# Xjh-UCAS/TAM-TR

Measured on AMD Instinct MI355X. Metric: images/sec fwd+bwd @640x640 bs=16/GPU, higher is better.
Workload: dtype bf16

## Files before the change

### tam-tr_amd/csrc/dwconv.hip

```cpp
#include "common.h"

namespace {

constexpr int TS = 16;
constexpr int DW_THREADS = TS * TS;
#ifndef DW_CB_BWD
#define DW_CB_BWD 16
#endif
constexpr int CB_FWD = 32, CB_BWD = DW_CB_BWD;

__device__ __forceinline__ float silu_f(float v) { return v / (1.f + __expf(-v)); }

template <typename T>
struct Vec16;
template <>
struct Vec16<float> {
  static constexpr int N = 4;
  static __device__ __forceinline__ void ld(const float* p, float (&o)[4]) {
    const float4 v = *reinterpret_cast<const float4*>(p);
    o[0] = v.x; o[1] = v.y; o[2] = v.z; o[3] = v.w;
  }
  static __device__ __forceinline__ void st(float* p, const float (&v)[4]) { *reinterpret_cast<float4*>(p) = make_float4(v[0], v[1], v[2], v[3]); }
};
template <>
struct Vec16<bf16_t> {
  static constexpr int N = 8;
  static __device__ __forceinline__ void ld(const bf16_t* p, float (&o)[8]) {
    const uint4 v = *reinterpret_cast<const uint4*>(p);
    const uint32_t w[4] = {v.x, v.y, v.z, v.w};
#pragma unroll
    for (int i = 0; i < 4; ++i) { o[2 * i] = __uint_as_float(w[i] << 16); o[2 * i + 1] = __uint_as_float(w[i] & 0xffff0000u); }
  }
  static __device__ __forceinline__ void st(bf16_t* p, const float (&v)[8]) {
    uint4 o;
    o.x = (uint32_t)f2bf(v[0]) | ((uint32_t)f2bf(v[1]) << 16); o.y = (uint32_t)f2bf(v[2]) | ((uint32_t)f2bf(v[3]) << 16);
    o.z = (uint32_t)f2bf(v[4]) | ((uint32_t)f2bf(v[5]) << 16); o.w = (uint32_t)f2bf(v[6]) | ((uint32_t)f2bf(v[7]) << 16);
    *reinterpret_cast<uint4*>(p) = o;
  }
};

__device__ __forceinline__ void plane_st(float* p, float v) { *p = v; }
__device__ __forceinline__ void plane_st(bf16_t* p, float v) { *p = f2bf(v); }
__device__ __forceinline__ float plane_ld(const float* p) { return *p; }
__device__ __forceinline__ float plane_ld(const bf16_t* p) { return bf2f(*p); }
__device__ __forceinline__ float4 plane_ld4(const float* p) { return *reinterpret_cast<const float4*>(p); }
__device__ __forceinline__ float4 plane_ld4(const bf16_t* p) {
  const uint2 v = *reinterpret_cast<const uint2*>(p);
  return make_float4(__uint_as_float(v.x << 16), __uint_as_float(v.x & 0xffff0000u), __uint_as_float(v.y << 16), __uint_as_float(v.y & 0xffff0000u));
}

template <typename T, int CB, int HALO, int PITCH>
__device__ __forceinline__ void stage_tile(const T* __restrict__ x, size_t xs, int b, int d0, int h0, int w0, int H, int W,
                                           float (*s)[TS + 2 * HALO][PITCH]) {
  constexpr int SIDE = TS + 2 * HALO, VN = Vec16<T>::N, GROUPS = CB / VN, TOTAL = SIDE * SIDE * GROUPS;
  constexpr int N_IT = (TOTAL + DW_THREADS - 1) / DW_THREADS;
  float v[N_IT][VN];
#pragma unroll
  for (int k = 0; k < N_IT; ++k) {
    const int it = min((int)threadIdx.x + k * DW_THREADS, TOTAL - 1);
    const int pix = it / GROUPS, gq = it - pix * GROUPS;
    const int py = pix / SIDE, px = pix - py * SIDE;
    const int h = min(max(h0 + py - HALO, 0), H - 1), w = min(max(w0 + px - HALO, 0), W - 1);
    Vec16<T>::ld(x + ((size_t)(b * H + h) * W + w) * xs + d0 + gq * VN, v[k]);
  }
#pragma unroll
  for (int k = 0; k < N_IT; ++k) {
    const int it = threadIdx.x + k * DW_THREADS;
    if (it < TOTAL) {
      const int pix = it / GROUPS, gq = it - pix * GROUPS;
      const int py = pix / SIDE, px = pix - py * SIDE;
      const int h = h0 + py - HALO, w = w0 + px - HALO;
      const float keep = (h >= 0 && h < H && w >= 0 && w < W) ? 1.f : 0.f;
#pragma unroll
      for (int j = 0; j < VN; ++j) s[gq * VN + j][py][px] = v[k][j] * keep;
    }
  }
}

template <typename T, typename PT>
__global__ __launch_bounds__(DW_THREADS) void dwconv_cross_fwd_kernel(const T* __restrict__ x, size_t xs, const float* __restrict__ wgt,
                                                                       const float* __restrict__ bias, PT* __restrict__ u2, int D,
                                                                       int H, int W, int tiles_w) {
  constexpr int CB = CB_FWD, SIDE = TS + 2, PITCH = SIDE + 1;
  __shared__ float s_in[CB][SIDE][PITCH];
  __shared__ float s_w[CB][10];
  const int th = blockIdx.x / tiles_w, tw = blockIdx.x - th * tiles_w;
  const int d0 = blockIdx.y * CB, b = blockIdx.z, h0 = th * TS, w0 = tw * TS;
  const size_t L = (size_t)H * W;
  for (int i = threadIdx.x; i < CB * 10; i += DW_THREADS) {
    const int c = i / 10, k = i - c * 10;
    s_w[c][k] = k < 9 ? wgt[(size_t)(d0 + c) * 9 + k] : (bias ? bias[d0 + c] : 0.f);
  }
  stage_tile<T, CB, 1, PITCH>(x, xs, b, d0, h0, w0, H, W, s_in);
  __syncthreads();
#pragma unroll
  for (int pass = 0; pass < 2; ++pass) {
    const int ty = pass == 0 ? threadIdx.x / TS : threadIdx.x % TS;
    const int tx = pass == 0 ? threadIdx.x % TS : threadIdx.x / TS;
    const int h = h0 + ty, w = w0 + tx;
    if (h >= H || w >= W) continue;
    PT* out = u2 + ((size_t)(b * 2 + pass) * D + d0) * L + (pass == 0 ? (size_t)h * W + w : (size_t)w * H + h);
    for (int c = 0; c < CB; ++c) {
      float acc = s_w[c][9];
#pragma unroll
      for (int ky = 0; ky < 3; ++ky)
#pragma unroll
        for (int kx = 0; kx < 3; ++kx) acc = fmaf(s_w[c][ky * 3 + kx], s_in[c][ty + ky][tx + kx], acc);
      plane_st(out + (size_t)c * L, silu_f(acc));
    }
  }
}

template <typename T, typename PT>
__global__ __launch_bounds__(DW_THREADS) void dwconv_cross_bwd_kernel(const PT* __restrict__ g2, const T* __restrict__ x, size_t xs,
                                                                       const float* __restrict__ wgt, const float* __restrict__ bias,
                                                                       T* __restrict__ gx, size_t gxs, float* __restrict__ ws, int D,
                                                                       int H, int W, int tiles_w, int tiles) {
  constexpr int CB = CB_BWD, XS = TS + 4, XP = XS + 1, GS = TS + 2, GP = GS + 1;
  __shared__ float s_x[CB][XS][XP];
  __shared__ float s_g[CB][GS][GP];
  __shared__ float s_w[CB][10];
  const int th = blockIdx.x / tiles_w, tw = blockIdx.x - th * tiles_w;
  const int d0 = blockIdx.y * CB, b = blockIdx.z, h0 = th * TS, w0 = tw * TS;
  const size_t L = (size_t)H * W;
  for (int i = threadIdx.x; i < CB * 10; i += DW_THREADS) {
    const int c = i / 10, k = i - c * 10;
    s_w[c][k] = k < 9 ? wgt[(size_t)(d0 + c) * 9 + k] : (bias ? bias[d0 + c] : 0.f);
  }
#ifndef DW_ABL_NOX
  stage_tile<T, CB, 2, XP>(x, xs, b, d0, h0, w0, H, W, s_x);
#endif
#ifndef DW_ABL_NOG
  if ((W & 3) == 0 && (H & 3) == 0) {
    constexpr int NV = 6, ITEMS_V = CB * GS * NV, N_ITV = (ITEMS_V + DW_THREADS - 1) / DW_THREADS;
#pragma unroll
    for (int plane = 0; plane < 2; ++plane) {
      const PT* gp = g2 + ((size_t)(b * 2 + plane) * D + d0) * L;
      float4 v[N_ITV];
#pragma unroll
      for (int k = 0; k < N_ITV; ++k) {
        const int it = min((int)threadIdx.x + k * DW_THREADS, ITEMS_V - 1);
        const int c = it / (GS * NV), r = it - c * (GS * NV), line = r / NV, q = r - line * NV;
        const int fixed = (plane == 0 ? h0 : w0) + line - 1, base = (plane == 0 ? w0 : h0) - 4 + 4 * q;
        const int nfix = plane == 0 ? H : W, nrun = plane == 0 ? W : H;
        const bool ok = fixed >= 0 && fixed < nfix && base >= 0 && base + 3 < nrun;
        const float4 t = plane_ld4(gp + (size_t)c * L + (size_t)min(max(fixed, 0), nfix - 1) * nrun + min(max(base, 0), nrun - 4));
        const float f = ok ? 1.f : 0.f;
        v[k] = make_float4(t.x * f, t.y * f, t.z * f, t.w * f);
      }
      if (plane == 1) __syncthreads();
#pragma unroll
      for (int k = 0; k < N_ITV; ++k) {
        const int it = threadIdx.x + k * DW_THREADS;
        if (it < ITEMS_V) {
          const int c = it / (GS * NV), r = it - c * (GS * NV), line = r / NV, q = r - line * NV;
          const float e[4] = {v[k].x, v[k].y, v[k].z, v[k].w};
#pragma unroll
          for (int j = 0; j < 4; ++j) {
            const int pos = 4 * q + j - 3;
            if (pos >= 0 && pos < GS) {
              if (plane == 0) s_g[c][line][pos] = e[j];
              else s_g[c][pos][line] += e[j];
            }
          }
        }
      }
    }
  } else {
  {
    constexpr int GB = 7, N_IT = ((CB * GS * GS + DW_THREADS - 1) / DW_THREADS + GB - 1) / GB * GB;
    const PT* gp = g2 + ((size_t)(b * 2 + 0) * D + d0) * L;
#pragma unroll 1
    for (int k0 = 0; k0 < N_IT; k0 += GB) {
      float v[GB];
#pragma unroll
      for (int k = 0; k < GB; ++k) {
        const int it = min((int)threadIdx.x + (k0 + k) * DW_THREADS, CB * GS * GS - 1);
        const int c = it / (GS * GS), r = it - c * (GS * GS), py = r / GS, px = r - py * GS;
        const int h = h0 + py - 1, w = w0 + px - 1;
        const bool ok = h >= 0 && h < H && w >= 0 && w < W;
        v[k] = plane_ld(gp + (size_t)c * L + (size_t)min(max(h, 0), H - 1) * W + min(max(w, 0), W - 1)) * (ok ? 1.f : 0.f);
      }
#pragma unroll
      for (int k = 0; k < GB; ++k) {
        const int it = threadIdx.x + (k0 + k) * DW_THREADS;
        if (it < CB * GS * GS) {
          const int c = it / (GS * GS), r = it - c * (GS * GS), py = r / GS, px = r - py * GS;
          s_g[c][py][px] = v[k];
        }
      }
    }
  }
  __syncthreads();
  {
    constexpr int GB = 7, N_IT = ((CB * GS * GS + DW_THREADS - 1) / DW_THREADS + GB - 1) / GB * GB;
    const PT* gp = g2 + ((size_t)(b * 2 + 1) * D + d0) * L;
#pragma unroll 1
    for (int k0 = 0; k0 < N_IT; k0 += GB) {
      float v[GB];
#pragma unroll
      for (int k = 0; k < GB; ++k) {
        const int it = min((int)threadIdx.x + (k0 + k) * DW_THREADS, CB * GS * GS - 1);
        const int c = it / (GS * GS), r = it - c * (GS * GS), px = r / GS, py = r - px * GS;
        const int h = h0 + py - 1, w = w0 + px - 1;
        const bool ok = h >= 0 && h < H && w >= 0 && w < W;
        v[k] = plane_ld(gp + (size_t)c * L + (size_t)min(max(w, 0), W - 1) * H + min(max(h, 0), H - 1)) * (ok ? 1.f : 0.f);
      }
#pragma unroll
      for (int k = 0; k < GB; ++k) {
        const int it = threadIdx.x + (k0 + k) * DW_THREADS;
        if (it < CB * GS * GS) {
          const int c = it / (GS * GS), r = it - c * (GS * GS), px = r / GS, py = r - px * GS;
          s_g[c][py][px] += v[k];
        }
      }
    }
  }
  }
#endif
  __syncthreads();
#ifndef DW_ABL_NOSILU
  {
    constexpr int TPC = DW_THREADS / CB;
    static_assert(DW_THREADS % CB == 0 && TPC <= WAVE && (TPC & (TPC - 1)) == 0, "a power-of-two lane group per channel");
    const int c = threadIdx.x / TPC, sub = threadIdx.x % TPC;
    float wk[9], dwk[10];
#pragma unroll
    for (int k9 = 0; k9 < 9; ++k9) { wk[k9] = s_w[c][k9]; dwk[k9] = 0.f; }
    dwk[9] = 0.f;
    const float bc = s_w[c][9];
    for (int r = sub; r < GS * GS; r += TPC) {
      const int px = r / GS, py = r - px * GS;
      const int h = h0 + py - 1, w = w0 + px - 1;
      float g = 0.f;
      if (h >= 0 && h < H && w >= 0 && w < W) {
        g = s_g[c][py][px];
        float xin[9], acc = bc;
#pragma unroll
        for (int ky = 0; ky < 3; ++ky)
#pragma unroll
          for (int kx = 0; kx < 3; ++kx) { xin[ky * 3 + kx] = s_x[c][py + ky][px + kx]; acc = fmaf(wk[ky * 3 + kx], xin[ky * 3 + kx], acc); }
        const float sg = 1.f / (1.f + __expf(-acc));
        g *= sg * (1.f + acc * (1.f - sg));
        if (py >= 1 && py <= TS && px >= 1 && px <= TS) {
#pragma unroll
          for (int k9 = 0; k9 < 9; ++k9) dwk[k9] = fmaf(g, xin[k9], dwk[k9]);
          dwk[9] += g;
        }
      }
      s_g[c][py][px] = g;
    }
#pragma unroll
    for (int k9 = 0; k9 < 10; ++k9) dwk[k9] = group_sum<TPC>(dwk[k9]);
    if (sub == 0) {
      float* o = ws + (((size_t)b * tiles + blockIdx.x) * D + d0 + c) * 10;
#pragma unroll
      for (int k9 = 0; k9 < 10; ++k9) o[k9] = dwk[k9];
    }
  }
#endif
  __syncthreads();
  const int ty = threadIdx.x / TS, tx = threadIdx.x % TS;
  float dxv[CB];
#pragma unroll
  for (int c = 0; c < CB; ++c) {
    float acc = 0.f;
#pragma unroll
    for (int ky = 0; ky < 3; ++ky)
#pragma unroll
      for (int kx = 0; kx < 3; ++kx) acc = fmaf(s_w[c][ky * 3 + kx], s_g[c][ty + 2 - ky][tx + 2 - kx], acc);
    dxv[c] = acc;
  }
  __syncthreads();
#pragma unroll
  for (int c = 0; c < CB; ++c) s_x[c][ty][tx] = dxv[c];
  __syncthreads();
  constexpr int VN = Vec16<T>::N, GROUPS = CB / VN;
  for (int it = threadIdx.x; it < TS * TS * GROUPS; it += DW_THREADS) {
    const int pix = it / GROUPS, gq = it - pix * GROUPS, py = pix / TS, px = pix - py * TS;
    const int h = h0 + py, w = w0 + px;
    if (h < H && w < W) {
      float v[VN];
#pragma unroll
      for (int j = 0; j < VN; ++j) v[j] = s_x[gq * VN + j][py][px];
      Vec16<T>::st(gx + ((size_t)(b * H + h) * W + w) * gxs + d0 + gq * VN, v);
    }
  }
}

}

static int dwconv_check(const void* a, const void* b, const void* c, int B, int D, int H, int W, long long xs, int dtype) {
  if (!a || !b || !c || B <= 0 || D <= 0 || H <= 0 || W <= 0 || xs < D) return TAMTR_EINVAL;
  if (dtype != TAMTR_F32 && dtype != TAMTR_BF16) return TAMTR_EINVAL;
  const int vn = dtype == TAMTR_F32 ? 4 : 8;
  if (D % CB_FWD || xs % vn || B > 65535 || D / CB_BWD > 65535) return TAMTR_EUNSUP;
  return TAMTR_OK;
}

extern "C" int tamtr_dwconv_silu_cross_fwd(const void* x, long long x_pixel_stride, const float* weight, const float* bias, void* u2,
                                           int B, int D, int H, int W, int dtype, int plane_dtype, void* stream) {
  const int rc = dwconv_check(x, weight, u2, B, D, H, W, x_pixel_stride, dtype);
  if (rc) return rc;
  if (plane_dtype != TAMTR_F32 && !(plane_dtype == TAMTR_BF16 && dtype == TAMTR_BF16)) return TAMTR_EINVAL;
  const int tiles_w = (W + TS - 1) / TS, tiles_h = (H + TS - 1) / TS;
  const dim3 grid(tiles_w * tiles_h, D / CB_FWD, B);
  hipStream_t s = (hipStream_t)stream;
  if (dtype == TAMTR_F32)
    hipLaunchKernelGGL((dwconv_cross_fwd_kernel<float, float>), grid, dim3(DW_THREADS), 0, s, (const float*)x, (size_t)x_pixel_stride, weight, bias,
                       (float*)u2, D, H, W, tiles_w);
  else if (plane_dtype == TAMTR_F32)
    hipLaunchKernelGGL((dwconv_cross_fwd_kernel<bf16_t, float>), grid, dim3(DW_THREADS), 0, s, (const bf16_t*)x, (size_t)x_pixel_stride, weight,
                       bias, (float*)u2, D, H, W, tiles_w);
  else
    hipLaunchKernelGGL((dwconv_cross_fwd_kernel<bf16_t, bf16_t>), grid, dim3(DW_THREADS), 0, s, (const bf16_t*)x, (size_t)x_pixel_stride, weight,
                       bias, (bf16_t*)u2, D, H, W, tiles_w);
  return tamtr_launch_status();
}

extern "C" int tamtr_dwconv_tiles(int H, int W) { return ((W + TS - 1) / TS) * ((H + TS - 1) / TS); }

extern "C" int tamtr_dwconv_silu_cross_bwd(const void* g2, const void* x, long long x_pixel_stride, const float* weight, const float* bias,
                                           void* gx, long long gx_pixel_stride, float* ws, int B, int D, int H, int W, int dtype,
                                           int plane_dtype, void* stream) {
  const int rc = dwconv_check(x, weight, g2, B, D, H, W, x_pixel_stride, dtype);
  if (rc) return rc;
  if (!gx || !ws || gx_pixel_stride < D || gx_pixel_stride % (dtype == TAMTR_F32 ? 4 : 8)) return TAMTR_EINVAL;
  if (plane_dtype != TAMTR_F32 && !(plane_dtype == TAMTR_BF16 && dtype == TAMTR_BF16)) return TAMTR_EINVAL;
  if ((uintptr_t)g2 % 16) return TAMTR_EUNSUP;
  const int tiles_w = (W + TS - 1) / TS, tiles_h = (H + TS - 1) / TS;
  const dim3 grid(tiles_w * tiles_h, D / CB_BWD, B);
  hipStream_t s = (hipStream_t)stream;
  if (dtype == TAMTR_F32)
    hipLaunchKernelGGL((dwconv_cross_bwd_kernel<float, float>), grid, dim3(DW_THREADS), 0, s, (const float*)g2, (const float*)x, (size_t)x_pixel_stride,
                       weight, bias, (float*)gx, (size_t)gx_pixel_stride, ws, D, H, W, tiles_w, tiles_w * tiles_h);
  else if (plane_dtype == TAMTR_F32)
    hipLaunchKernelGGL((dwconv_cross_bwd_kernel<bf16_t, float>), grid, dim3(DW_THREADS), 0, s, (const float*)g2, (const bf16_t*)x,
                       (size_t)x_pixel_stride, weight, bias, (bf16_t*)gx, (size_t)gx_pixel_stride, ws, D, H, W, tiles_w, tiles_w * tiles_h);
  else
    hipLaunchKernelGGL((dwconv_cross_bwd_kernel<bf16_t, bf16_t>), grid, dim3(DW_THREADS), 0, s, (const bf16_t*)g2, (const bf16_t*)x,
                       (size_t)x_pixel_stride, weight, bias, (bf16_t*)gx, (size_t)gx_pixel_stride, ws, D, H, W, tiles_w, tiles_w * tiles_h);
  return tamtr_launch_status();
}
```

Before: 214.6.

## Compute depthwise conv on 2x2 output patches per lane with register windows

The forward and backward depthwise 3x3 conv kernels now give each lane a 2x2 output patch and load a 4x4 input window from shared memory with float2 reads. The shared-memory pitch changes to a fixed 20-float layout padded against bank conflicts. Weights are read straight from global memory into registers instead of a shared weight table, and each wave owns whole channels. The forward pass writes paired outputs for both planes when alignment allows. The backward SiLU/weight-grad stage is rebalanced across channel pairs with cross-half reductions, which adds register pressure and more complex indexing.

```diff
diff --git a/tam-tr_amd/csrc/dwconv.hip b/tam-tr_amd/csrc/dwconv.hip
--- a/tam-tr_amd/csrc/dwconv.hip
+++ b/tam-tr_amd/csrc/dwconv.hip
@@ -49,9 +49,22 @@
   return make_float4(__uint_as_float(v.x << 16), __uint_as_float(v.x & 0xffff0000u), __uint_as_float(v.y << 16), __uint_as_float(v.y & 0xffff0000u));
 }
 
-template <typename T, int CB, int HALO, int PITCH>
-__device__ __forceinline__ void stage_tile(const T* __restrict__ x, size_t xs, int b, int d0, int h0, int w0, int H, int W,
-                                           float (*s)[TS + 2 * HALO][PITCH]) {
+__device__ __forceinline__ void plane_st2(float* p, float a, float b) { *reinterpret_cast<float2*>(p) = make_float2(a, b); }
+__device__ __forceinline__ void plane_st2(bf16_t* p, float a, float b) { *reinterpret_cast<uint32_t*>(p) = (uint32_t)f2bf(a) | ((uint32_t)f2bf(b) << 16); }
+
+constexpr int TP = 20;
+__device__ __forceinline__ void patch_of_lane(int lane, int& pi, int& pj) { pj = lane & 7; pi = ((lane >> 3) & 3) * 2 + (lane >> 5); }
+
+__device__ __forceinline__ void ld_window(const float* sp, float (&o)[4][4]) {
+#pragma unroll
+  for (int r = 0; r < 4; ++r) {
+    const float2 a = *reinterpret_cast<const float2*>(sp + r * TP), c = *reinterpret_cast<const float2*>(sp + r * TP + 2);
+    o[r][0] = a.x; o[r][1] = a.y; o[r][2] = c.x; o[r][3] = c.y;
+  }
+}
+
+template <typename T, int CB, int HALO, int PITCH, int CS>
+__device__ __forceinline__ void stage_tile(const T* __restrict__ x, size_t xs, int b, int d0, int h0, int w0, int H, int W, float* s) {
   constexpr int SIDE = TS + 2 * HALO, VN = Vec16<T>::N, GROUPS = CB / VN, TOTAL = SIDE * SIDE * GROUPS;
   constexpr int N_IT = (TOTAL + DW_THREADS - 1) / DW_THREADS;
   float v[N_IT][VN];
@@ -72,7 +85,7 @@
       const int h = h0 + py - HALO, w = w0 + px - HALO;
       const float keep = (h >= 0 && h < H && w >= 0 && w < W) ? 1.f : 0.f;
 #pragma unroll
-      for (int j = 0; j < VN; ++j) s[gq * VN + j][py][px] = v[k][j] * keep;
+      for (int j = 0; j < VN; ++j) s[(gq * VN + j) * CS + py * PITCH + px] = v[k][j] * keep;
     }
   }
 }
@@ -80,34 +93,96 @@
 template <typename T, typename PT>
 __global__ __launch_bounds__(DW_THREADS) void dwconv_cross_fwd_kernel(const T* __restrict__ x, size_t xs, const float* __restrict__ wgt,
                                                                        const float* __restrict__ bias, PT* __restrict__ u2, int D,
-                                                                       int H, int W, int tiles_w) {
-  constexpr int CB = CB_FWD, SIDE = TS + 2, PITCH = SIDE + 1;
-  __shared__ float s_in[CB][SIDE][PITCH];
-  __shared__ float s_w[CB][10];
+                                                                       int H, int W, int tiles_w, int pair) {
+  constexpr int CB = CB_FWD, SIDE = TS + 2, CS = SIDE * TP + 2;
+  static_assert(SIDE <= TP && (8 * CS) % 64 == 16, "see the note on TP");
+  __shared__ __attribute__((aligned(16))) float s_in[CB * CS];
   const int th = blockIdx.x / tiles_w, tw = blockIdx.x - th * tiles_w;
   const int d0 = blockIdx.y * CB, b = blockIdx.z, h0 = th * TS, w0 = tw * TS;
   const size_t L = (size_t)H * W;
-  for (int i = threadIdx.x; i < CB * 10; i += DW_THREADS) {
-    const int c = i / 10, k = i - c * 10;
-    s_w[c][k] = k < 9 ? wgt[(size_t)(d0 + c) * 9 + k] : (bias ? bias[d0 + c] : 0.f);
-  }
-  stage_tile<T, CB, 1, PITCH>(x, xs, b, d0, h0, w0, H, W, s_in);
-  __syncthreads();
-#pragma unroll
-  for (int pass = 0; pass < 2; ++pass) {
-    const int ty = pass == 0 ? threadIdx.x / TS : threadIdx.x % TS;
-    const int tx = pass == 0 ? threadIdx.x % TS : threadIdx.x / TS;
-    const int h = h0 + ty, w = w0 + tx;
-    if (h >= H || w >= W) continue;
-    PT* out = u2 + ((size_t)(b * 2 + pass) * D + d0) * L + (pass == 0 ? (size_t)h * W + w : (size_t)w * H + h);
-    for (int c = 0; c < CB; ++c) {
-      float acc = s_w[c][9];
+  stage_tile<T, CB, 1, TP, CS>(x, xs, b, d0, h0, w0, H, W, s_in);
+  __syncthreads();
+  const int wv = __builtin_amdgcn_readfirstlane(threadIdx.x / WAVE);
+  int pi, pj;
+  patch_of_lane(threadIdx.x % WAVE, pi, pj);
+  const int h = h0 + 2 * pi, w = w0 + 2 * pj;
+  if (h >= H || w >= W) return;
+  const bool h1 = h + 1 < H, w1 = w + 1 < W;
+  for (int c = wv; c < CB; c += DW_THREADS / WAVE) {
+    float wk[9];
+#pragma unroll
+    for (int k = 0; k < 9; ++k) wk[k] = wgt[(size_t)(d0 + c) * 9 + k];
+    const float bc = bias ? bias[d0 + c] : 0.f;
+    float in[4][4], o[2][2];
+    ld_window(s_in + c * CS + 2 * pi * TP + 2 * pj, in);
+#pragma unroll
+    for (int dy = 0; dy < 2; ++dy)
+#pragma unroll
+      for (int dx = 0; dx < 2; ++dx) {
+        float acc = bc;
+#pragma unroll
+        for (int ky = 0; ky < 3; ++ky)
+#pragma unroll
+          for (int kx = 0; kx < 3; ++kx) acc = fmaf(wk[ky * 3 + kx], in[dy + ky][dx + kx], acc);
+        o[dy][dx] = silu_f(acc);
+      }
+    PT* p0 = u2 + ((size_t)(b * 2 + 0) * D + d0 + c) * L + (size_t)h * W + w;
+    PT* p1 = u2 + ((size_t)(b * 2 + 1) * D + d0 + c) * L + (size_t)w * H + h;
+    if (pair & 1) {
+      plane_st2(p0, o[0][0], o[0][1]);
+      if (h1) plane_st2(p0 + W, o[1][0], o[1][1]);
+    } else {
+      plane_st(p0, o[0][0]);
+      if (w1) plane_st(p0 + 1, o[0][1]);
+      if (h1) {
+        plane_st(p0 + W, o[1][0]);
+        if (w1) plane_st(p0 + W + 1, o[1][1]);
+      }
+    }
+    if (pair & 2) {
+      plane_st2(p1, o[0][0], o[1][0]);
+      if (w1) plane_st2(p1 + H, o[0][1], o[1][1]);
+    } else {
+      plane_st(p1, o[0][0]);
+      if (h1) plane_st(p1 + 1, o[1][0]);
+      if (w1) {
+        plane_st(p1 + H, o[0][1]);
+        if (h1) plane_st(p1 + H + 1, o[1][1]);
+      }
+    }
+  }
+}
+
+__device__ __forceinline__ void silu_bwd_patch(const float* sx, float* sg, int pi, int pj, bool act, const float (&w)[10], int hb, int wb,
+                                               int H, int W, float (&dwk)[10]) {
+  float in[4][4];
+  ld_window(sx + 2 * pi * TP + 2 * pj, in);
+  float* gp = sg + 2 * pi * TP + 2 * pj;
+  const float2 g0 = *reinterpret_cast<const float2*>(gp), g1 = *reinterpret_cast<const float2*>(gp + TP);
+  float g[2][2] = {{g0.x, g0.y}, {g1.x, g1.y}};
+#pragma unroll
+  for (int dy = 0; dy < 2; ++dy)
+#pragma unroll
+    for (int dx = 0; dx < 2; ++dx) {
+      const int py = 2 * pi + dy, px = 2 * pj + dx, h = hb + py, wp = wb + px;
+      float acc = w[9];
 #pragma unroll
       for (int ky = 0; ky < 3; ++ky)
 #pragma unroll
-        for (int kx = 0; kx < 3; ++kx) acc = fmaf(s_w[c][ky * 3 + kx], s_in[c][ty + ky][tx + kx], acc);
-      plane_st(out + (size_t)c * L, silu_f(acc));
-    }
+        for (int kx = 0; kx < 3; ++kx) acc = fmaf(w[ky * 3 + kx], in[dy + ky][dx + kx], acc);
+      const float sgm = 1.f / (1.f + __expf(-acc));
+      const float gv = (h >= 0 && h < H && wp >= 0 && wp < W) ? g[dy][dx] * (sgm * (1.f + acc * (1.f - sgm))) : 0.f;
+      g[dy][dx] = gv;
+      const float gc = (act && py >= 1 && py <= TS && px >= 1 && px <= TS) ? gv : 0.f;
+#pragma unroll
+      for (int ky = 0; ky < 3; ++ky)
+#pragma unroll
+        for (int kx = 0; kx < 3; ++kx) dwk[ky * 3 + kx] = fmaf(gc, in[dy + ky][dx + kx], dwk[ky * 3 + kx]);
+      dwk[9] += gc;
+    }
+  if (act) {
+    *reinterpret_cast<float2*>(gp) = make_float2(g[0][0], g[0][1]);
+    *reinterpret_cast<float2*>(gp + TP) = make_float2(g[1][0], g[1][1]);
   }
 }
 
@@ -116,19 +191,16 @@
                                                                        const float* __restrict__ wgt, const float* __restrict__ bias,
                                                                        T* __restrict__ gx, size_t gxs, float* __restrict__ ws, int D,
                                                                        int H, int W, int tiles_w, int tiles) {
-  constexpr int CB = CB_BWD, XS = TS + 4, XP = XS + 1, GS = TS + 2, GP = GS + 1;
-  __shared__ float s_x[CB][XS][XP];
-  __shared__ float s_g[CB][GS][GP];
-  __shared__ float s_w[CB][10];
+  constexpr int CB = CB_BWD, XS = TS + 4, XP = TP, CSX = XS * XP + 4, GS = TS + 2, GP = TP, CSG = GS * GP;
+  constexpr int NW = DW_THREADS / WAVE;
+  static_assert(XS <= TP && (8 * CSX) % 64 == 32 && CB % (2 * NW) == 0, "see the note on TP; a wave works on pairs of channels");
+  __shared__ __attribute__((aligned(16))) float s_x[CB * CSX];
+  __shared__ __attribute__((aligned(16))) float s_g[CB * CSG];
   const int th = blockIdx.x / tiles_w, tw = blockIdx.x - th * tiles_w;
   const int d0 = blockIdx.y * CB, b = blockIdx.z, h0 = th * TS, w0 = tw * TS;
   const size_t L = (size_t)H * W;
-  for (int i = threadIdx.x; i < CB * 10; i += DW_THREADS) {
-    const int c = i / 10, k = i - c * 10;
-    s_w[c][k] = k < 9 ? wgt[(size_t)(d0 + c) * 9 + k] : (bias ? bias[d0 + c] : 0.f);
-  }
 #ifndef DW_ABL_NOX
-  stage_tile<T, CB, 2, XP>(x, xs, b, d0, h0, w0, H, W, s_x);
+  stage_tile<T, CB, 2, XP, CSX>(x, xs, b, d0, h0, w0, H, W, s_x);
 #endif
 #ifndef DW_ABL_NOG
   if ((W & 3) == 0 && (H & 3) == 0) {
@@ -159,8 +231,8 @@
           for (int j = 0; j < 4; ++j) {
             const int pos = 4 * q + j - 3;
             if (pos >= 0 && pos < GS) {
-              if (plane == 0) s_g[c][line][pos] = e[j];
-              else s_g[c][pos][line] += e[j];
+              if (plane == 0) s_g[c * CSG + line * GP + pos] = e[j];
+              else s_g[c * CSG + pos * GP + line] += e[j];
             }
           }
         }
@@ -186,7 +258,7 @@
         const int it = threadIdx.x + (k0 + k) * DW_THREADS;
         if (it < CB * GS * GS) {
           const int c = it / (GS * GS), r = it - c * (GS * GS), py = r / GS, px = r - py * GS;
-          s_g[c][py][px] = v[k];
+          s_g[c * CSG + py * GP + px] = v[k];
         }
       }
     }
@@ -211,7 +283,7 @@
         const int it = threadIdx.x + (k0 + k) * DW_THREADS;
         if (it < CB * GS * GS) {
           const int c = it / (GS * GS), r = it - c * (GS * GS), px = r / GS, py = r - px * GS;
-          s_g[c][py][px] += v[k];
+          s_g[c * CSG + py * GP + px] += v[k];
         }
       }
     }
@@ -219,61 +291,66 @@
   }
 #endif
   __syncthreads();
+  const int lane = threadIdx.x % WAVE, wv = __builtin_amdgcn_readfirstlane(threadIdx.x / WAVE);
+  int pi, pj;
+  patch_of_lane(lane, pi, pj);
 #ifndef DW_ABL_NOSILU
   {
-    constexpr int TPC = DW_THREADS / CB;
-    static_assert(DW_THREADS % CB == 0 && TPC <= WAVE && (TPC & (TPC - 1)) == 0, "a power-of-two lane group per channel");
-    const int c = threadIdx.x / TPC, sub = threadIdx.x % TPC;
-    float wk[9], dwk[10];
-#pragma unroll
-    for (int k9 = 0; k9 < 9; ++k9) { wk[k9] = s_w[c][k9]; dwk[k9] = 0.f; }
-    dwk[9] = 0.f;
-    const float bc = s_w[c][9];
-    for (int r = sub; r < GS * GS; r += TPC) {
-      const int px = r / GS, py = r - px * GS;
-      const int h = h0 + py - 1, w = w0 + px - 1;
-      float g = 0.f;
-      if (h >= 0 && h < H && w >= 0 && w < W) {
-        g = s_g[c][py][px];
-        float xin[9], acc = bc;
+    const int l32 = lane & 31, half = lane >> 5;
+    const bool ract = l32 < 17;
+    const int ri = l32 < 9 ? 8 : min(l32 - 9, 7), rj = l32 < 9 ? l32 : 8;
+    for (int q = wv; q < CB / 2; q += NW) {
+      const int c0 = 2 * q;
+      float wk[2][10], wr[10], dwk[3][10];
+#pragma unroll
+      for (int e = 0; e < 2; ++e) {
+#pragma unroll
+        for (int k9 = 0; k9 < 9; ++k9) wk[e][k9] = wgt[(size_t)(d0 + c0 + e) * 9 + k9];
+        wk[e][9] = bias ? bias[d0 + c0 + e] : 0.f;
+      }
+#pragma unroll
+      for (int k9 = 0; k9 < 10; ++k9) { wr[k9] = half ? wk[1][k9] : wk[0][k9]; dwk[0][k9] = dwk[1][k9] = dwk[2][k9] = 0.f; }
+      silu_bwd_patch(s_x + c0 * CSX, s_g + c0 * CSG, pi, pj, true, wk[0], h0 - 1, w0 - 1, H, W, dwk[0]);
+      silu_bwd_patch(s_x + (c0 + 1) * CSX, s_g + (c0 + 1) * CSG, pi, pj, true, wk[1], h0 - 1, w0 - 1, H, W, dwk[1]);
+      silu_bwd_patch(s_x + (c0 + half) * CSX, s_g + (c0 + half) * CSG, ri, rj, ract, wr, h0 - 1, w0 - 1, H, W, dwk[2]);
+      float* o = ws + (((size_t)b * tiles + blockIdx.x) * D + d0 + c0 + half) * 10;
+#pragma unroll
+      for (int k9 = 0; k9 < 10; ++k9) {
+        const float mine = half ? dwk[1][k9] : dwk[0][k9], other = half ? dwk[0][k9] : dwk[1][k9];
+        const float v = group_sum<32>(mine + dwk[2][k9] + __shfl_xor(other, 32, WAVE));
+        if (l32 == 0) o[k9] = v;
+      }
+    }
+  }
+#endif
+  __syncthreads();
+  float dxv[CB / NW][2][2];
+#pragma unroll
+  for (int k = 0; k < CB / NW; ++k) {
+    const int c = wv + NW * k;
+    float wk[9], gw[4][4];
+#pragma unroll
+    for (int k9 = 0; k9 < 9; ++k9) wk[k9] = wgt[(size_t)(d0 + c) * 9 + k9];
+    ld_window(s_g + c * CSG + 2 * pi * GP + 2 * pj, gw);
+#pragma unroll
+    for (int dy = 0; dy < 2; ++dy)
+#pragma unroll
+      for (int dx = 0; dx < 2; ++dx) {
+        float acc = 0.f;
 #pragma unroll
         for (int ky = 0; ky < 3; ++ky)
 #pragma unroll
-          for (int kx = 0; kx < 3; ++kx) { xin[ky * 3 + kx] = s_x[c][py + ky][px + kx]; acc = fmaf(wk[ky * 3 + kx], xin[ky * 3 + kx], acc); }
-        const float sg = 1.f / (1.f + __expf(-acc));
-        g *= sg * (1.f + acc * (1.f - sg));
-        if (py >= 1 && py <= TS && px >= 1 && px <= TS) {
-#pragma unroll
-          for (int k9 = 0; k9 < 9; ++k9) dwk[k9] = fmaf(g, xin[k9], dwk[k9]);
-          dwk[9] += g;
-        }
-      }
-      s_g[c][py][px] = g;
-    }
-#pragma unroll
-    for (int k9 = 0; k9 < 10; ++k9) dwk[k9] = group_sum<TPC>(dwk[k9]);
-    if (sub == 0) {
-      float* o = ws + (((size_t)b * tiles + blockIdx.x) * D + d0 + c) * 10;
-#pragma unroll
-      for (int k9 = 0; k9 < 10; ++k9) o[k9] = dwk[k9];
-    }
-  }
-#endif
-  __syncthreads();
-  const int ty = threadIdx.x / TS, tx = threadIdx.x % TS;
-  float dxv[CB];
-#pragma unroll
-  for (int c = 0; c < CB; ++c) {
-    float acc = 0.f;
-#pragma unroll
-    for (int ky = 0; ky < 3; ++ky)
-#pragma unroll
-      for (int kx = 0; kx < 3; ++kx) acc = fmaf(s_w[c][ky * 3 + kx], s_g[c][ty + 2 - ky][tx + 2 - kx], acc);
-    dxv[c] = acc;
-  }
-  __syncthreads();
-#pragma unroll
-  for (int c = 0; c < CB; ++c) s_x[c][ty][tx] = dxv[c];
+          for (int kx = 0; kx < 3; ++kx) acc = fmaf(wk[ky * 3 + kx], gw[dy + 2 - ky][dx + 2 - kx], acc);
+        dxv[k][dy][dx] = acc;
+      }
+  }
+  __syncthreads();
+#pragma unroll
+  for (int k = 0; k < CB / NW; ++k) {
+    float* p = s_x + (wv + NW * k) * CSX + 2 * pi * XP + 2 * pj;
+    *reinterpret_cast<float2*>(p) = make_float2(dxv[k][0][0], dxv[k][0][1]);
+    *reinterpret_cast<float2*>(p + XP) = make_float2(dxv[k][1][0], dxv[k][1][1]);
+  }
   __syncthreads();
   constexpr int VN = Vec16<T>::N, GROUPS = CB / VN;
   for (int it = threadIdx.x; it < TS * TS * GROUPS; it += DW_THREADS) {
@@ -282,7 +359,7 @@
     if (h < H && w < W) {
       float v[VN];
 #pragma unroll
-      for (int j = 0; j < VN; ++j) v[j] = s_x[gq * VN + j][py][px];
+      for (int j = 0; j < VN; ++j) v[j] = s_x[(gq * VN + j) * CSX + py * XP + px];
       Vec16<T>::st(gx + ((size_t)(b * H + h) * W + w) * gxs + d0 + gq * VN, v);
     }
   }
@@ -306,15 +383,17 @@
   const int tiles_w = (W + TS - 1) / TS, tiles_h = (H + TS - 1) / TS;
   const dim3 grid(tiles_w * tiles_h, D / CB_FWD, B);
   hipStream_t s = (hipStream_t)stream;
+  const bool base_ok = (uintptr_t)u2 % (plane_dtype == TAMTR_F32 ? 8 : 4) == 0;
+  const int pair = (base_ok && W % 2 == 0 ? 1 : 0) | (base_ok && H % 2 == 0 ? 2 : 0);
   if (dtype == TAMTR_F32)
     hipLaunchKernelGGL((dwconv_cross_fwd_kernel<float, float>), grid, dim3(DW_THREADS), 0, s, (const float*)x, (size_t)x_pixel_stride, weight, bias,
-                       (float*)u2, D, H, W, tiles_w);
+                       (float*)u2, D, H, W, tiles_w, pair);
   else if (plane_dtype == TAMTR_F32)
     hipLaunchKernelGGL((dwconv_cross_fwd_kernel<bf16_t, float>), grid, dim3(DW_THREADS), 0, s, (const bf16_t*)x, (size_t)x_pixel_stride, weight,
-                       bias, (float*)u2, D, H, W, tiles_w);
+                       bias, (float*)u2, D, H, W, tiles_w, pair);
   else
     hipLaunchKernelGGL((dwconv_cross_fwd_kernel<bf16_t, bf16_t>), grid, dim3(DW_THREADS), 0, s, (const bf16_t*)x, (size_t)x_pixel_stride, weight,
-                       bias, (bf16_t*)u2, D, H, W, tiles_w);
+                       bias, (bf16_t*)u2, D, H, W, tiles_w, pair);
   return tamtr_launch_status();
 }
 
```

Measured after the change: 214.4. About the same (-0.1%).
